# peterrum/dealii-multigrid

Hardware: AMD Instinct MI355X
Metric: DoF/s per V-cycle, 3D octant p=4 (higher is better)
Workload: dtype f64; 1 GPU; 3D octant (GeometryType quadrant) HMG-global p=4 FP64, NRefGlobal=8, SmootherDegree=3, coarse solver direct, f=1, zero Dirichlet (BASELINE.json configs[2]); n_dofs=137199985, n_cells=2127189, n_levels=9, parallelism=1 GPU, chebyshev_start_vector=deal.II's (i mod 11) - mean on the local numbering, fused_transfer_bricks=33509

## Files before the change

### dealii_multigrid_amd/__init__.py

```python
from __future__ import annotations

import ctypes as C
import os

import numpy as np

_LIB_PATH = os.environ.get("MGAMD_LIBRARY") or os.path.join(os.path.dirname(os.path.abspath(__file__)), "lib", "libmgamd.so")
F64, F32 = 8, 4
AMG_MIN_SHARDED_ROWS_DEFAULT = 20000
INVALID_DOF = 0xFFFFFFFF
ALL_DIRICHLET = 0x3F


class MgamdError(RuntimeError):
    pass


class NoDeviceError(MgamdError):
    pass


def _load():
    if not os.path.exists(_LIB_PATH):
        raise MgamdError(
# ... 354 lines not shown
    def rhs_constant(self):
        b = np.zeros(self.n_dofs)
        _chk(_lib.mgamd_dofs_rhs_constant(self._h, _ptr(b)))
        return b

    def groups(self):
        return [(self.info.group_B[g], self.info.group_slots[g]) for g in range(self.info.n_groups)]

    def matrix(self):
        nnz = C.c_uint64()
        _chk(_lib.mgamd_dofs_matrix(self._h, C.byref(nnz), None, None, None))
        ptr, col, val = np.zeros(self.n_dofs + 1, np.uint32), np.zeros(nnz.value, np.uint32), np.zeros(nnz.value)
        _chk(_lib.mgamd_dofs_matrix(self._h, C.byref(nnz), _ptr(ptr), _ptr(col), _ptr(val)))
        return ptr, col, val

    def amg_setup_info(self):
        n, rows, nnz = C.c_uint32(), (C.c_uint32 * 32)(), (C.c_uint64 * 32)()
        _chk(_lib.mgamd_dofs_amg_setup_info(self._h, C.byref(n), rows, nnz, 32))
        return [(rows[l], nnz[l]) for l in range(n.value)]

    def amg_hierarchy(self) -> "AmgHostHierarchy":
        return AmgHostHierarchy(self)

    def cell_slots(self):
        grp, slot = np.zeros(self.info.n_cells, np.uint8), np.zeros(self.info.n_cells, np.uint32)
        _chk(_lib.mgamd_dofs_get_cell_slots(self._h, _ptr(grp), _ptr(slot)))
        return grp, slot

    def halo_plan(self):
        sz = (C.c_uint32 * 4)()
        _chk(_lib.mgamd_dofs_halo_sizes(self._h, sz))
        npeer, nsend, nsh, nc = (int(v) for v in sz)
        plan = dict(peers=np.zeros(npeer, np.int32), peer_offset=np.zeros(npeer + 1, np.uint32), pack_idx=np.zeros(nsend, np.uint32),
                    sh_tail=np.zeros(nsh, np.uint32), sh_ptr=np.zeros(nsh + 1, np.uint32), sh_src=np.zeros(nc, np.int32),
                    sh_owner_src=np.zeros(nsh, np.int32))
        if npeer:
            _chk(_lib.mgamd_dofs_halo_get(self._h, _ptr(plan["peers"]), _ptr(plan["peer_offset"]), _ptr(plan["pack_idx"]), _ptr(plan["sh_tail"]),
                                          _ptr(plan["sh_ptr"]), _ptr(plan["sh_src"]), _ptr(plan["sh_owner_src"])))
        return plan

    def __del__(self):
        if getattr(self, "_h", None) and _lib is not None:
            _lib.mgamd_dofs_destroy(self._h)
            self._h = None


# ... 216 lines not shown
    def rhs_boundary_flux(self, b: Vector, q):
        q = _flux_array(q)
        _chk(_lib.mgamd_level_op_rhs_boundary_flux(self._h, _ptr(q), b._h))

    def distribute(self, x: Vector, kind: int = 0):
        _chk(_lib.mgamd_level_op_distribute(self._h, kind, x._h))

    def rhs_dirichlet(self, b: Vector, g: Vector, include_mass: bool = True):
        _chk(_lib.mgamd_level_op_rhs_dirichlet(self._h, g._h, 1 if include_mass else 0, b._h))

    def distribute_values(self, x: Vector, g: Vector):
        _chk(_lib.mgamd_level_op_distribute_values(self._h, x._h, g._h))

    def estimate_error(self, u: Vector, q=None):
        eta = np.zeros(self.dofs.info.n_cells, np.float64)
        qa = None if q is None else _flux_array(q)
        _chk(_lib.mgamd_level_op_estimate_error(self._h, u._h, None if qa is None else _ptr(qa), _ptr(eta)))
        return eta

    def _estimator_info(self):
        b, t0, t1 = C.c_uint64(), C.c_double(), C.c_double()
        _chk(_lib.mgamd_debug_level_op_estimator_info(self._h, C.byref(b), C.byref(t0), C.byref(t1)))
        return b.value, t0.value, t1.value

    def get_system_matrix(self) -> "SparseMatrix":
        if self.dofs.mass_coefficient() != self.mass_coefficient():
            raise MgamdError(f"get_system_matrix: the mass coefficient of the DoFs ({self.dofs.mass_coefficient()}) was changed after this "
                             f"operator was built with {self.mass_coefficient()}; the assembled matrix would be another operator's")
        return SparseMatrix(self.ctx, self.dofs)

    def __del__(self):
        if getattr(self, "_h", None) and _lib is not None:
            _lib.mgamd_level_op_destroy(self._h)
            self._h = None


class PreconditionChebyshev:
    def __init__(self, op: Operator, degree=3, smoothing_range=20.0, eig_cg_n_iterations=20):
        self.op = op
        self._h = C.c_void_p()
        _chk(_lib.mgamd_cheb_create(op._h, degree, C.c_double(smoothing_range), eig_cg_n_iterations, C.byref(self._h)))

    def vmult(self, dst: Vector, src: Vector):
        _chk(_lib.mgamd_cheb_vmult(self._h, dst._h, src._h))

    def step(self, dst: Vector, src: Vector):
# ... 519 lines not shown
```

### dealii_multigrid_amd/csrc/c_api_device.hip

```cpp
#include "runtime.hpp"
#include "kernels_amg.hpp"
#include <cstdio>

using namespace mgamd;

#define REQUIRE(cond)                                    \
  if (!(cond))                                           \
  throw std::invalid_argument("null or invalid argument: " #cond)

extern "C" {

int
mgamd_ctx_create(int device, mgamd_ctx **out)
{
  MGAMD_TRY
  REQUIRE(out);
  auto *c = new mgamd_ctx;
  try
    {
      c->ctx = std::make_unique<Ctx>(device);
    }
  catch (...)
    {
      delete c;
// ... 426 lines not shown
int
mgamd_level_op_estimate_error(mgamd_level_op *op, const mgamd_vec *u, const double q[6], double *eta)
{
  MGAMD_TRY
  REQUIRE(op && u);
  op->op->estimate_error(*u, q, eta);
  MGAMD_CATCH
}

int
mgamd_debug_level_op_estimator_info(const mgamd_level_op *op, uint64_t *bytes, double *build_ms, double *kernel_ms)
{
  MGAMD_TRY
  REQUIRE(op);
  uint64_t b  = 0;
  double   t0 = 0.0, t1 = 0.0;
  op->op->estimator_info(b, t0, t1);
  if (bytes)
    *bytes = b;
  if (build_ms)
    *build_ms = t0;
  if (kernel_ms)
    *kernel_ms = t1;
  MGAMD_CATCH
}

int
mgamd_level_op_debug_stamps(mgamd_level_op *op, unsigned long long *out, uint64_t max_count, uint64_t *count)
{
  MGAMD_TRY
  REQUIRE(op && out && count);
  *count = op->op->read_debug_stamps(out, max_count);
  MGAMD_CATCH
}

int
mgamd_cheb_create(mgamd_level_op *op, unsigned degree, double smoothing_range, unsigned eig_cg_n_iterations, mgamd_cheb **out)
{
  MGAMD_TRY
  REQUIRE(op && out);
  auto *h = new mgamd_cheb;
  try
    {
      h->c.reset(make_chebyshev(op->op.get(), degree, smoothing_range, eig_cg_n_iterations));
    }
  catch (...)
// ... 720 lines not shown
```

### dealii_multigrid_amd/csrc/c_api_host.cpp

```cpp
#include "api_common.hpp"

using namespace mgamd;

namespace mgamd
{
  thread_local std::string g_last_error;
}

struct mgamd_amg_host
{
  AmgHierarchyHost H;
};

struct mgamd_amg_shard
{
  AmgHierarchyHost          H;
  unsigned                  n_sharded = 0;
  std::vector<AmgShardPlan> plans;
};

extern "C" {

const char *
mgamd_last_error(void)
// ... 800 lines not shown
  std::vector<uint32_t> g, l;
  ls_copy_indices(*active_mesh_dofs->tables, *level_dofs->tables, (int)level, g, l);
  *count = g.size();
  if (global_idx)
    std::copy(g.begin(), g.end(), global_idx);
  if (level_idx)
    std::copy(l.begin(), l.end(), level_idx);
  MGAMD_CATCH
}

int
mgamd_dofs_get_cell_slots(const mgamd_dofs *d, uint8_t *group, uint32_t *slot)
{
  MGAMD_TRY
  if (!d || !group || !slot)
    throw std::invalid_argument("null argument");
  const LevelTables &L = *d->tables;
  std::copy(L.cell_group.begin(), L.cell_group.end(), group);
  std::copy(L.cell_slot.begin(), L.cell_slot.end(), slot);
  MGAMD_CATCH
}

int
mgamd_dofs_get_keys(const mgamd_dofs *d, int32_t *keys)
{
  MGAMD_TRY
  if (!d || !keys)
    throw std::invalid_argument("null argument");
  std::vector<DofKey> k;
  d->tables->export_dof_keys(k);
  static_assert(sizeof(DofKey) == 5 * sizeof(int32_t), "DofKey layout");
  std::memcpy(keys, k.data(), k.size() * sizeof(DofKey));
  MGAMD_CATCH
}

int
mgamd_dofs_get_cell_dofs(const mgamd_dofs *d, uint32_t *out)
{
  MGAMD_TRY
  if (!d || !out)
    throw std::invalid_argument("null argument");
  std::vector<uint32_t> v;
  d->tables->export_cell_dofs(v);
  std::memcpy(out, v.data(), v.size() * sizeof(uint32_t));
  MGAMD_CATCH
}
// ... 264 lines not shown
```

### dealii_multigrid_amd/csrc/kernels_apply.hpp

```cpp
#pragma once
#include "kernels_common.hpp"

namespace mgamd
{
#ifdef MGAMD_KERNEL_DEBUG
#define MGAMD_STAMP(k)                         \
  if (args.stamps && tid == 0)                 \
    args.stamps[(size_t)block * 8 + (k)] = wall_clock64();
#define MGAMD_ABLATED(bit) (args.ablate & (bit))
#define MGAMD_STAMP_OWNER(w)                   \
  if (args.stamps && tid == 0)                 \
    args.stamps[(size_t)block * 8 + 7] = (w) + 1;
#else
#define MGAMD_STAMP(k)
#define MGAMD_STAMP_OWNER(w)
#define MGAMD_ABLATED(bit) false
#endif

  template <typename T, int P>
  __device__ __forceinline__ void
  interior_diag_terms(const Mats<P, T> &mats, const int t, T &s_K, T &s_M)
  {
    const int tt[3] = {t % P, (t / P) % P, t / (P * P)};
    T         m[3], k[3];
// ... 337 lines not shown
        return (x % P) + P * ((y % P) + P * (z % P));
      }
      __device__ __forceinline__ void
      next()
      {
        constexpr int DZ = BLOCK / (NI * NI), DY = (BLOCK % (NI * NI)) / NI, DX = BLOCK % NI;
        x += DX;
        if (x > NI)
          {
            x -= NI;
            ++y;
          }
        y += DY;
        if (y > NI)
          {
            y -= NI;
            ++z;
          }
        z += DZ;
      }
    };
    const InteriorWalk walk0{tid % NI + 1, (tid / NI) % NI + 1, tid / (NI * NI) + 1};
    auto has_entry = [&](int it) -> bool { return (it + 1) * BLOCK <= G::N_INT || tid + it * BLOCK < G::N_INT; };
    int spos[ITERS];
#pragma unroll
    for (int it = 0; it < ITERS; ++it)
      {
        const int idx = tid + it * BLOCK;
        spos[it]      = idx < G::N_SHELL ? (int)args.g.shell_pos[idx] : -1;
      }
    if (sched.active && tid == 0)
      sched.publish(drawn, ticket_word);
    __syncthreads();

    constexpr bool x_from_b = MODE == MODE_CHEB_FIRST;
    auto load_tables = [&](uint32_t s, uint32_t &slot, uint32_t &base, uint32_t(&sg)[ITERS], double &h, uint32_t &fm, uint32_t &fl,
                           uint32_t(&cg)[ITC]) {
      slot = s;
      base = args.g.interior_base[slot];
      h    = args.g.h[slot];
      fm   = 0;
      fl   = 0;
      if constexpr (FUSE)
        {
          fl = args.fused.flags[(size_t)slot * BLOCK + tid];
          const uint32_t *__restrict__ c0 = args.fused.coarse_idx + (size_t)slot * NC3;
#pragma unroll
          for (int it = 0; it < ITC; ++it)
            cg[it] = NT_LOAD(c0 + min(tid + it * BLOCK, NC3 - 1));
        }
      if constexpr (brick_may_be_constrained(B, CONSTR))
        if (args.g.fmask != nullptr)
          fm = args.g.fmask[slot];
      const uint32_t *__restrict__ p0 = args.g.shell_idx + (size_t)slot * G::N_SHELL;
#pragma unroll
      for (int it = 0; it < ITERS; ++it)
        {
          if ((it + 1) * BLOCK <= G::N_SHELL)
            sg[it] = NT_LOAD(p0 + it * BLOCK + tid);
          else
            sg[it] = NT_LOAD(p0 + min(tid + it * BLOCK, G::N_SHELL - 1));
        }
    };
    auto load_values = [&](uint32_t base, const uint32_t(&sg)[ITERS], const uint32_t fl, const uint32_t(&cg)[ITC], T(&xv)[ITER], T(&sv)[ITERS],
                           T(&sbv)[ITERS], T(&cv)[ITC]) {
      const T *__restrict__ in = x_from_b ? args.epi.b : args.src;
#pragma unroll
      for (int it = 0; it < ITER; ++it)
        xv[it] = NT_LOAD(&in[base + (uint32_t)(has_entry(it) ? tid + it * BLOCK : 0)]);
#pragma unroll
      for (int it = 0; it < ITERS; ++it)
        {
          const uint32_t gi = sg[it] < args.gather_limit ? sg[it] : 0;
          sv[it]            = in[gi];
          if (x_from_b)
            sbv[it] = args.epi.dinv[gi];
          if (FUSE_R)
            sbv[it] = args.epi.b[((fl >> (2 * it)) & 1u) ? gi : 0];
        }
      if constexpr (FUSE_P)
        {
#pragma unroll
          for (int it = 0; it < ITC; ++it)
            cv[it] = args.fused.coarse[cg[it] != DEV_INVALID ? cg[it] : 0];
        }
    };

    uint32_t slot, base, sgi[ITERS], fmcur, flcur, cgi[ITC];
    double   hcur;
    T        xg[ITER], sval[ITERS], sb[ITERS], cval[ITC];
    load_tables(xcd_contiguous(w, n), slot, base, sgi, hcur, fmcur, flcur, cgi);
    load_values(base, sgi, flcur, cgi, xg, sval, sb, cval);

    for (;;)
      {
        const uint32_t block = slot;
        (void)block;
        uint32_t   vn       = slot;
        const bool has_next = sched.active && sched.take(ticket_word, vn);
        if (has_next && tid == 0)
          drawn = sched.draw();
        MGAMD_STAMP(0)
        MGAMD_STAMP_OWNER(w)
        const T rh = T(1) / T(hcur);
        if constexpr (MASS && is_cheb(MODE))
          {
            const T c = T(args.sigma) * T(args.g.q[slot]);
            for (int t = tid; t < P3; t += BLOCK)
              {
                T s_K, s_M;
                interior_diag_terms<T, P>(args.m, t, s_K, s_M);
                const T sv   = s_K + c * s_M;
                dtab[t]      = sv;
                dtab[P3 + t] = T(1) / sv;
              }
            if (x_from_b)
              __syncthreads();
          }
        auto interior_dinv = [&](int t) -> T {
          return fabs((double)dtab[t]) > 1.0e-10 * fabs((double)rh) ? rh * dtab[P3 + t] : T(1);
        };
        const bool fused_slot = FUSE && ((__builtin_amdgcn_readfirstlane((int)flcur) >> 15) & 1);
        T          bv[ITER], xo[ITER];
        uint32_t slotn = slot, basen = base, sgn[ITERS], fmn = fmcur, fln = flcur, cgn[ITC];
        double   hn = hcur;
        if (has_next)
          load_tables(vn, slotn, basen, sgn, hn, fmn, fln, cgn);
        {
#pragma unroll
          for (int it = 0; it < ITER; ++it)
            {
              const uint32_t g = base + (uint32_t)(has_entry(it) ? tid + it * BLOCK : 0);
              xo[it]           = T(0);
              bv[it]           = x_from_b ? xg[it] : T(0);
              if (MODE == MODE_CHEB && !FUSE_P && args.epi.xold)
                xo[it] = NT_LOAD(&args.epi.xold[g]);
              if ((MODE == MODE_RESIDUAL || is_cheb(MODE)) && !x_from_b)
                bv[it] = NT_LOAD(&args.epi.b[g]);
            }
        }
        if constexpr (FUSE_P)
          if (fused_slot)
            {
#pragma unroll
              for (int it = 0; it < ITC; ++it)
                if (tid + it * BLOCK < NC3)
                  bufA[tid + it * BLOCK] = ((flcur >> (16 + it)) & 1u) ? T(0) : cval[it];
              __syncthreads();
              T cin[NC], cout[G::N];
              for (int l = tid; l < NC * NC; l += BLOCK)
// ... 14 lines not shown
#pragma unroll
                  for (int i = 0; i < NC; ++i)
                    cin[i] = bufB[b0 + i * G::N];
                  line_embed_sym<T, P, BC>(args.fused.Eh, cin, cout);
#pragma unroll
                  for (int i = 0; i < G::N; ++i)
                    bufB[b0 + i * G::N] = cout[i];
                }
              __syncthreads();
              for (int l = tid; l < G::N * G::N; l += BLOCK)
                {
                  const int b0 = l * G::N;
#pragma unroll
                  for (int i = 0; i < NC; ++i)
                    cin[i] = bufB[b0 + i];
                  line_embed_sym<T, P, BC>(args.fused.Eh, cin, cout);
#pragma unroll
                  for (int i = 0; i < G::N; ++i)
                    bufB[b0 + i] = cout[i];
                }
              __syncthreads();
#pragma unroll
              for (int it = 0; it < ITERS; ++it)
                if (spos[it] >= 0 && sgi[it] < args.gather_limit)
                  {
                    const uint32_t f2 = (flcur >> (2 * it)) & 3u;
                    if (!(f2 & 2u))
                      sval[it] += bufB[spos[it]];
                    if (f2 & 1u)
                      args.fused.scratch[sgi[it]] = sval[it];
                  }
              InteriorWalk wk = walk0;
#pragma unroll
              for (int it = 0; it < ITER; ++it, wk.next())
                if (has_entry(it))
                  {
                    xg[it] += bufB[wk.pos()];
                    NT_STORE(xg[it], &args.fused.x_inout[base + (uint32_t)(tid + it * BLOCK)]);
                  }
            }
        if (x_from_b)
          {
#pragma unroll
            for (int it = 0; it < ITERS; ++it)
              sval[it] = args.epi.c0 * sb[it] * sval[it];
          }
#pragma unroll
        for (int it = 0; it < ITERS; ++it)
          if (spos[it] >= 0)
            bufA[spos[it]] = sgi[it] < args.gather_limit ? sval[it] : T(0);
        {
          InteriorWalk wk = walk0;
#pragma unroll
          for (int it = 0; it < ITER; ++it, wk.next())
            if (has_entry(it))
              bufA[wk.pos()] = x_from_b ? args.epi.c0 * interior_dinv(wk.type()) * bv[it] : xg[it];
        }
        __syncthreads();
        if (has_next && tid == 0)
          sched.publish(drawn, ticket_word);
        MGAMD_STAMP(1)

        bool any_hanging = false;
        if constexpr (brick_may_be_constrained(B, CONSTR))
          {
            any_hanging = fmcur != 0;
            if (any_hanging)
              brick_constraint_passes<T, P, B, BLOCK>(bufA, args.m, tid, 1, args.g.fmask + slot, false, &fmcur);
          }
        if constexpr (MODE == MODE_MASS)
          mass_sweeps<T, P, B, BLOCK, true, true, false>(bufA, args.m, tid, 1, &hcur, false);
        else
          lattice_sweeps<T, P, B, BLOCK, NoHook, true, (MODE != MODE_CHEB || sizeof(T) == 4), false, MASS>(
            bufA, bufB, args.m, tid, 1, &hcur, NoHook(), false, args.sigma, args.g.q + slot);
        if constexpr (brick_may_be_constrained(B, CONSTR))
          if (any_hanging)
            brick_constraint_passes<T, P, B, BLOCK>(bufA, args.m, tid, 1, args.g.fmask + slot, true, &fmcur);
        MGAMD_STAMP(2)

        T xgn[ITER], svaln[ITERS], sbn[ITERS], cvaln[ITC];
        if (has_next)
          load_values(basen, sgn, fln, cgn, xgn, svaln, sbn, cvaln);

        if (FUSE_R && fused_slot)
          {
            if constexpr (FUSE_R)
              {
                InteriorWalk wk = walk0;
#pragma unroll
                for (int it = 0; it < ITER; ++it, wk.next())
                  if (has_entry(it))
                    bufA[wk.pos()] = bv[it] - bufA[wk.pos()];
#pragma unroll
                for (int it = 0; it < ITERS; ++it)
                  if (spos[it] >= 0)
                    bufA[spos[it]] = sgi[it] < args.scatter_limit ? (((flcur >> (2 * it)) & 1u) ? sb[it] : T(0)) - bufA[spos[it]] : T(0);
                __syncthreads();
                T rin[G::N], rout[NC];
                for (int l = tid; l < G::N * G::N; l += BLOCK)
                  {
                    const int b0 = l * G::N;
#pragma unroll
                    for (int i = 0; i < G::N; ++i)
                      rin[i] = bufA[b0 + i];
                    line_embed_sym_T<T, P, BC>(args.fused.Eh, rin, rout);
#pragma unroll
                    for (int i = 0; i < NC; ++i)
                      bufA[b0 + i] = rout[i];
                  }
                __syncthreads();
                for (int l = tid; l < NC * G::N; l += BLOCK)
                  {
                    const int b0 = (l / NC) * G::N * G::N + l % NC;
#pragma unroll
                    for (int i = 0; i < G::N; ++i)
                      rin[i] = bufA[b0 + i * G::N];
                    line_embed_sym_T<T, P, BC>(args.fused.Eh, rin, rout);
#pragma unroll
                    for (int i = 0; i < NC; ++i)
// ... 30 lines not shown
                  T              r;
                  if (MODE == MODE_VMULT || MODE == MODE_MASS)
                    r = ax;
                  else if (MODE == MODE_RESIDUAL)
                    r = bv[it] - ax;
                  else
                    {
                      const T dv  = interior_dinv(wk.type());
                      const T xov = MODE == MODE_CHEB_SECOND ? args.epi.c0 * dv * bv[it] : xo[it];
                      const T xv  = x_from_b ? args.epi.c0 * dv * bv[it] : xg[it];
                      if (FUSE_P)
                        r = xv + args.epi.f2 * dv * (bv[it] - ax);
                      else
                        r = xv + args.epi.f1 * (xv - xov) + args.epi.f2 * dv * (bv[it] - ax);
                    }
                  if (MODE == MODE_CHEB && !FUSE_P)
                    store_result(args.epi, g, r);
                  else
                    NT_STORE(r, &args.epi.out[g]);
                }
            MGAMD_STAMP(3)
#pragma unroll
            for (int it = 0; it < ITERS; ++it)
              if (spos[it] >= 0 && sgi[it] < args.scatter_limit)
                atomic_add(&args.tail_acc[sgi[it] - args.n_interior], bufA[spos[it]]);
          }
        MGAMD_STAMP(4)
        if (!has_next)
          break;
        slot  = slotn;
        base  = basen;
        hcur  = hn;
        fmcur = fmn;
        flcur = fln;
#pragma unroll
        for (int it = 0; it < ITC; ++it)
          {
            cgi[it]  = cgn[it];
            cval[it] = cvaln[it];
          }
#pragma unroll
        for (int it = 0; it < ITERS; ++it)
          {
            sgi[it]  = sgn[it];
            sval[it] = svaln[it];
            sb[it]   = sbn[it];
          }
#pragma unroll
// ... 878 lines not shown
```

### dealii_multigrid_amd/csrc/kernels_common.hpp

```cpp
#pragma once
#include <hip/hip_runtime.h>
#include <stdint.h>

namespace mgamd
{
  constexpr uint32_t DEV_INVALID = 0xFFFFFFFFu;

  constexpr size_t KERNARG_LIMIT     = 4096;
  constexpr int    MAX_KERNEL_DEGREE = 7;

#ifndef MGAMD_NO_NT_STREAMS
#define NT_LOAD(p) __builtin_nontemporal_load(p)
#define NT_STORE(v, p) __builtin_nontemporal_store(v, p)
#else
#define NT_LOAD(p) (*(p))
#define NT_STORE(v, p) (*(p) = (v))
#endif

  __device__ __forceinline__ uint32_t
  xcd_contiguous(uint32_t b, uint32_t n)
  {
    const uint32_t k = b & 7u, q = n >> 3, r = n & 7u;
    return k * q + (k < r ? k : r) + (b >> 3);
  }
// ... 76 lines not shown
  persistent_brick(int p)
  {
    return 16 % p == 0 ? 16 / p : 0;
  }
  template <typename T, int P, int B>
  constexpr size_t
  apply_lds_bytes()
  {
    using G = Geo<P, B>;
    static_assert(persistent_lattice(G::N) == (G::SPW == 1 && G::N_INT > 0 && G::ROUNDS > 1), "persistent_lattice() and Geo disagree");
    return (2 * (size_t)G::SPW * G::N3 + 2 * P * P * P * (P == 1 ? G::SPW : 1) + G::SPW) * sizeof(T);
  }

  struct SlotGroupDev
  {
    const uint32_t *interior_base;
    const uint32_t *shell_idx;
    const uint16_t *mask;
    const double   *h;
    const uint16_t *shell_pos;
    uint32_t        n_slots;
    const uint32_t *fmask;
    const double   *q;
  };

  enum ApplyMode
  {
    MODE_VMULT    = 0,
    MODE_RESIDUAL = 1,
    MODE_CHEB     = 2,
    MODE_INVDIAG  = 3,
    MODE_CHEB_FIRST  = 4,
    MODE_CHEB_SECOND = 5,
    MODE_RESIDUAL_RESTRICT = 6,
    MODE_CHEB_PROLONGATE = 7,
    MODE_MASS = 8
  };
  constexpr int
  base_mode(int mode)
  {
    return mode == MODE_RESIDUAL_RESTRICT ? MODE_RESIDUAL : (mode == MODE_CHEB_PROLONGATE ? MODE_CHEB : mode);
  }

  template <typename T>
  struct Epilogue
  {
    T       *out;
// ... 1046 lines not shown
```

### dealii_multigrid_amd/csrc/level_operator.hpp

```cpp
#pragma once
#include "runtime.hpp"
#include "kernels.hpp"

#include <chrono>
#include <cmath>
#include <cstring>
#include <map>
#include <mutex>
#include <type_traits>
#include <unordered_map>

namespace mgamd
{
  inline int
  grid_for(size_t n)
  {
    size_t g = (n + 255) / 256;
    if (g > 2048)
      g = 2048;
    if (g < 1)
      g = 1;
    return (int)g;
  }

// ... 96 lines not shown
      }
    else if constexpr (persistent_lattice(G::N))
      {
        void (*kern)(ApplyArgs<T, P>) = lattice_apply_persistent_kernel<T, P, B, MODE, CONSTR, false>;
        if constexpr (MODE != MODE_MASS)
          if (a.sigma != 0.0)
            kern = lattice_apply_persistent_kernel<T, P, B, MODE, CONSTR, true>;
        launch_persistent(ctx, st, kern, grid, persistent_wgs_per_cu<T, P>(), G::ABLOCK, apply_lds_bytes<T, P, B>(), a, grid_cap);
      }
    else
      launch_lds(ctx, st, lattice_apply_kernel<T, P, B, MODE, CONSTR>, grid, G::ABLOCK, apply_lds_bytes<T, P, B>(), a);
    HIP_CHECK(hipGetLastError());
  }

  template <typename T>
  struct GroupDev
  {
    int            B = 1, N = 2;
    bool           constrained = false;
    size_t         n_halo      = 0;
    size_t         n_slots = 0;
    DBuf<uint32_t> interior_base, shell_idx;
    DBuf<uint16_t> mask, shell_pos;
    DBuf<double>   h, q, h_cell;
    DBuf<uint32_t> fmask;
    void
    upload_scales(const SlotGroup &g)
    {
      std::vector<double> ah(g.h.size()), ratio(g.h.size());
      bool                any = false;
      for (size_t s = 0; s < g.h.size(); ++s)
        {
          ah[s]    = g.a[s] * g.h[s];
          ratio[s] = g.h[s] * g.h[s] / g.a[s];
          any |= g.a[s] != 1.0;
        }
      h.upload(ah);
      q.upload(ratio);
      if (any)
        h_cell.upload(g.h);
    }
    const double *
    scale(bool mass_pass) const
    {
      return mass_pass && h_cell.p ? h_cell.p : h.p;
    }
    SlotGroupDev
    view(bool mass_pass) const
    {
      return SlotGroupDev{interior_base.p, shell_idx.p, mask.p, scale(mass_pass), shell_pos.p, (uint32_t)n_slots, fmask.p, q.p};
    }
    SlotGroupDev
    view(size_t begin, size_t end, bool mass_pass) const
    {
      const size_t n_shell = (size_t)N * N * N - (size_t)(N - 2) * (N - 2) * (N - 2);
      return SlotGroupDev{interior_base.p + begin, shell_idx.p + begin * n_shell, mask.p + begin, scale(mass_pass) + begin, shell_pos.p,
                          (uint32_t)(end - begin), fmask.p ? fmask.p + begin : nullptr, q.p + begin};
    }
    DBuf<uint32_t> uniq_ptr, uniq_idx;
    DBuf<uint16_t> loc;
    uint32_t       max_uniq = 0;
    bool
    has_clusters() const
    {
      return uniq_ptr.p != nullptr;
    }
    CellClusterDev
    cluster_view(bool mass_pass) const
    {
      return CellClusterDev{uniq_ptr.p, uniq_idx.p, loc.p, mask.p, scale(mass_pass), (uint32_t)n_slots, max_uniq, q.p};
    }
    size_t
    cluster_lds_bytes() const
    {
      return 2 * (size_t)std::max<uint32_t>(max_uniq, 1) * sizeof(T);
    }
    void
    build_clusters(const SlotGroup &g)
    {
      const size_t          ns = g.n_slots(), ncl = (ns + CLUSTER_CELLS - 1) / CLUSTER_CELLS;
// ... 161 lines not shown
          halo->sh_tail.upload(halo_plan->sh_tail);
          halo->sh_ptr.upload(halo_plan->sh_ptr);
          halo->sh_src.upload(halo_plan->sh_src);
          halo->sh_owner_src.upload(halo_plan->sh_owner_src);
          halo->send.alloc(std::max<size_t>(halo_plan->pack_idx.size(), 1));
          halo->recv.alloc(std::max<size_t>(halo_plan->pack_idx.size(), 1));
        }
      size_t best = 0;
      for (const SlotGroup &g : tables->groups)
        {
          auto d     = std::make_unique<GroupDev<T>>();
          d->B           = g.B;
          d->N           = g.N;
          d->constrained = g.constrained_group;
          d->n_halo      = g.n_halo_slots;
          d->n_slots = g.n_slots();
          if (d->n_slots)
            {
              d->interior_base.upload(g.interior_base);
              d->shell_idx.upload(g.shell_idx);
              d->mask.upload(g.mask);
              d->upload_scales(g);
              d->shell_pos.upload(g.shell_pos);
              if (std::any_of(g.fmask.begin(), g.fmask.end(), [](uint32_t m) { return m != 0; }))
                d->fmask.upload(g.fmask);
              if (p == 1 && g.B == 1 && !tables->ls_level)
                d->build_clusters(g);
            }
          const size_t work = d->n_slots * (size_t)g.N * g.N * g.N;
          if (work > best)
            {
              best       = work;
              dominant_B = g.B;
            }
          groups.push_back(std::move(d));
        }
      if (const char *e = getenv("MGAMD_ABLATE"))
        ablate = (uint32_t)atoi(e);
      if (const char *e = getenv("MGAMD_STAMP_B"))
        dominant_B = atoi(e);
      halo_overlap = getenv("MGAMD_NO_HALO_OVERLAP") == nullptr;
      if (const char *e = getenv("MGAMD_STAMPS"))
        {
          stamp_mode = atoi(e);
          size_t nwg = 0;
          for (auto &g : groups)
// ... 736 lines not shown
      float ms = 0.f;
      HIP_CHECK(hipEventElapsedTime(&ms, estimator->e0, estimator->e1));
      estimator->kernel_ms = ms;
    }
    void
    estimator_info(uint64_t &bytes, double &build_ms, double &kernel_ms) const override
    {
      bytes     = estimator ? estimator->bytes : 0;
      build_ms  = estimator ? estimator->build_ms : 0.0;
      kernel_ms = estimator ? estimator->kernel_ms : 0.0;
    }

    size_t
    read_debug_stamps(unsigned long long *out, size_t max_count) override
    {
      ctx->sync();
      const size_t n = std::min(max_count, stamps.n);
      if (n)
        HIP_CHECK(hipMemcpy(out, stamps.p, n * sizeof(unsigned long long), hipMemcpyDeviceToHost));
      return n;
    }

    void
    compute_inverse_diagonal(mgamd_vec &d) override
    {
      if (d.n != n_dofs())
        throw std::invalid_argument("compute_inverse_diagonal: vector size mismatch");
      Epilogue<T> e{d.as<T>(), nullptr, nullptr, nullptr, nullptr, T(0), T(0)};
      apply<MODE_VMULT>(nullptr, e, true);
    }
  };

}
```

### dealii_multigrid_amd/csrc/level_tables.hpp

```cpp
#pragma once
#include <algorithm>
#include <array>
#include <cmath>
#include <cstdlib>
#include <cstring>
#include "fe1d.hpp"
#include "octree.hpp"

#include <map>

namespace mgamd
{
  struct SharedInfo
  {
    uint64_t others  = 0;
    uint64_t regular = 0;
  };
  inline int
  shared_owner(const SharedInfo &si)
  {
    return __builtin_ctzll(si.regular);
  }
}

// ... 31 lines not shown
    s += M * N;
    if (y == N - 1)
      return s + (z - 1) * N + x;
    s += M * N;
    if (x == 0)
      return s + (z - 1) * M + (y - 1);
    s += M * M;
    return s + (z - 1) * M + (y - 1);
  }

  struct SlotGroup
  {
    int                   B = 1, N = 2, n_interior = 0, n_shell = 8;
    std::vector<uint32_t> interior_base;
    std::vector<uint32_t> shell_idx;
    std::vector<uint16_t> mask;
    std::vector<uint32_t> fmask;
    std::vector<double>   h;
    std::vector<double>   a;
    std::vector<uint32_t> first_cell;
    std::vector<uint16_t> shell_pos;
    uint32_t n_halo_slots = 0;
    bool constrained_group = false;
    size_t
    n_slots() const
    {
      return interior_base.size();
    }
  };

  struct DofKey
  {
    int32_t px, py, pz, dirmask, level;
  };

  inline uint64_t
  pack_key(uint32_t px, uint32_t py, uint32_t pz, int dm, int level)
  {
    return ((uint64_t)px << 43) | ((uint64_t)py << 25) | ((uint64_t)pz << 7) | ((uint64_t)dm << 4) | (uint64_t)(dm ? level : 0);
  }
  inline DofKey
  unpack_key(uint64_t k)
  {
    return DofKey{(int32_t)(k >> 43), (int32_t)((k >> 25) & 0x3ffff), (int32_t)((k >> 7) & 0x3ffff), (int32_t)((k >> 4) & 7),
                  (int32_t)(k & 15)};
  }

  inline void
  interpolate_hanging(const FE1D &fe, uint16_t mask, double *v, bool transpose)
  {
    if (!(mask >> MASK_FACE_SHIFT))
      return;
// ... 1281 lines not shown
                  perm.push_back((uint32_t)sl);
              auto permute = [&](auto &v, size_t width) {
                if (v.empty())
                  return;
                auto old = v;
                for (size_t n2 = 0; n2 < ns; ++n2)
                  std::copy(old.begin() + perm[n2] * width, old.begin() + (perm[n2] + 1) * width, v.begin() + n2 * width);
              };
              permute(g.interior_base, 1);
              permute(g.shell_idx, (size_t)g.n_shell);
              permute(g.mask, 1);
              permute(g.fmask, 1);
              permute(g.h, 1);
              permute(g.a, 1);
              permute(g.first_cell, 1);
              std::vector<uint32_t> new_of_old(ns);
              for (size_t n2 = 0; n2 < ns; ++n2)
                new_of_old[perm[n2]] = (uint32_t)n2;
              for (size_t ci = 0; ci < nc; ++ci)
                if (cell_group[ci] == gi)
                  cell_slot[ci] = new_of_old[cell_slot[ci]];
            }
        }
      build_robin_faces();
      build_dirichlet_cells();
    }

    void
    dirichlet_lift_add(const double *g, bool include_mass, double alpha, std::vector<double> &b) const
    {
      const int           n = p + 1, n3 = n * n * n;
      std::vector<double> xg(n3), lift(n3);
      for (size_t e = 0; e < dirichlet_cells.size(); ++e)
        {
          const uint32_t *idx = &dirichlet_cells.idx[e * n3];
          for (int t = 0; t < n3; ++t)
            xg[t] = is_dirichlet_index(idx[t]) ? g[idx[t]] : 0.0;
          const uint16_t mask = dirichlet_cells.mask[e];
          const double   ah = dirichlet_cells.scale[2 * e], h = dirichlet_cells.scale[2 * e + 1];
          interpolate_hanging(fe, mask, xg.data(), false);
          cell_stiffness_apply(ah, xg.data(), lift.data());
          if (include_mass && sigma != 0.0)
            cell_mass_add(h, sigma, xg.data(), lift.data());
          interpolate_hanging(fe, mask, lift.data(), true);
          for (int t = 0; t < n3; ++t)
            if (idx[t] < first_constrained())
// ... 82 lines not shown
```

### dealii_multigrid_amd/csrc/runtime.hpp

```cpp
#pragma once
#include "api_common.hpp"
#include "comm.hpp"

#include <hip/hip_runtime.h>

#include <functional>
#include <map>
#include <sstream>

namespace mgamd
{
#define HIP_CHECK(expr)                                                                                       \
  do                                                                                                          \
    {                                                                                                         \
      hipError_t e_ = (expr);                                                                                 \
      if (e_ != hipSuccess)                                                                                   \
        {                                                                                                     \
          std::ostringstream os_;                                                                             \
          os_ << "HIP error " << hipGetErrorString(e_) << " at " << __FILE__ << ":" << __LINE__ << ": " #expr; \
          throw std::runtime_error(os_.str());                                                                \
        }                                                                                                     \
    }                                                                                                         \
  while (0)

// ... 156 lines not shown
    }
    uint32_t
    n_dofs() const
    {
      return tables->n_dofs;
    }
    size_t
    n_dot() const
    {
      return comm ? (size_t)tables->n_interior + tables->n_tail_owned : (size_t)n_dofs();
    }
    virtual void
    vmult(mgamd_vec &dst, const mgamd_vec &src) = 0;
    virtual void
    vmult_mass(mgamd_vec &dst, const mgamd_vec &src) = 0;
    virtual void
    compute_inverse_diagonal(mgamd_vec &d) = 0;
    virtual void
    vmult_interface_up(mgamd_vec &dst, const mgamd_vec &src) = 0;
    virtual void
    vmult_interface_down(mgamd_vec &dst, const mgamd_vec &src) = 0;
    virtual size_t
    read_debug_stamps(unsigned long long *out, size_t max_count) = 0;
    void
    rhs(mgamd_vec &b, int kind = 0);
    void
    rhs_boundary_flux(mgamd_vec &b, const double q[6]);
    void
    distribute(mgamd_vec &x, int kind);
    virtual void
    rhs_dirichlet(mgamd_vec &rhs, const mgamd_vec &g, bool include_mass) = 0;
    virtual void
    distribute_values(mgamd_vec &x, const mgamd_vec &g) = 0;
    virtual void
    estimate_error(const mgamd_vec &u, const double *q, double *eta) = 0;
    virtual void
    estimator_info(uint64_t &bytes, double &build_ms, double &kernel_ms) const = 0;

  private:
    virtual void
    distribute_values_core(mgamd_vec &x, const mgamd_vec &g) = 0;
    void
    upload_load(mgamd_vec &b, const std::vector<double> &h);
  };

  struct ChebyshevBase
// ... 189 lines not shown
```

### include/mgamd_dev.h

```cpp
#ifndef MGAMD_DEV_H
#define MGAMD_DEV_H

#include "mgamd.h"

#ifdef __cplusplus
extern "C" {
#endif

int mgamd_level_op_debug_stamps(mgamd_level_op *op, unsigned long long *out, uint64_t max_count, uint64_t *count);

int mgamd_ctx_kernel_profile(mgamd_ctx *ctx, int enable);
int mgamd_ctx_kernel_profile_brick(mgamd_ctx *ctx, int brick_size);
int mgamd_ctx_kernel_profile_read(mgamd_ctx *ctx, double *total_ms, uint64_t *n_launches, double *algorithmic_bytes);
int mgamd_ctx_kernel_profile_bytes_moved(mgamd_ctx *ctx, double *bytes_moved);

int mgamd_debug_coarse_resolve(const char *name, uint64_t n_level0_dofs, int level0_sharded, int has_nested, int has_amg_global,
                               char used[32]);

typedef struct mgamd_amg_host mgamd_amg_host;
int mgamd_debug_amg_host_create(const mgamd_dofs *d, mgamd_amg_host **out);
int mgamd_debug_amg_host_destroy(mgamd_amg_host *h);
int mgamd_debug_amg_host_n_levels(const mgamd_amg_host *h, uint32_t *n_levels);
int mgamd_debug_amg_host_level_info(const mgamd_amg_host *h, uint32_t level, uint32_t *n_rows, uint64_t *nnz_A, uint32_t *n_cols_P,
                                    uint64_t *nnz_P, uint32_t *n_aggregates, double *lambda_max);
// ... 7 lines not shown
int mgamd_debug_amg_shard_match_rows(const mgamd_dofs *global, const mgamd_dofs *local, uint32_t *rows);
int mgamd_debug_amg_shard_n_levels(const mgamd_amg_shard *h, uint32_t *n_levels, uint32_t *n_sharded_levels);
int mgamd_debug_amg_shard_level_info(const mgamd_amg_shard *h, unsigned rank, uint32_t level, uint32_t info[12]);
int mgamd_debug_amg_shard_level_get(const mgamd_amg_shard *h, unsigned rank, uint32_t level, uint32_t *rows, uint32_t *ghost, int32_t *peers,
                                    uint32_t *peer_offset, uint32_t *send_count, uint32_t *recv_count, uint32_t *send_idx, uint32_t *A_ptr,
                                    uint32_t *A_col, double *A_val, uint32_t *P_ptr, uint32_t *P_col, double *P_val, uint32_t *R_ptr,
                                    uint32_t *R_col, double *R_val);

int mgamd_debug_csr_spmv(mgamd_ctx *ctx, int number_type, int mode, int lanes, uint32_t n_rows, uint32_t n_cols, const uint32_t *ptr,
                         const uint32_t *col, const double *val, const double *x, double *y, const double *b, const double *xold,
                         int xold_is_y, const double *dinv, double f1, double f2, int *lanes_used);

int mgamd_debug_csr_spmv_ex(mgamd_ctx *ctx, int number_type, int mode, int lanes, uint32_t n_rows, uint32_t n_cols, const uint32_t *ptr,
                            const uint32_t *col, const double *val, const double *x, double *y, const double *b, const double *xold,
                            int xold_is_y, const double *dinv, double f1, double f2, int max_blocks, int *lanes_used, int *blocks,
                            double *dot);
int mgamd_debug_csr_spmv_lanes_long(uint32_t n_rows, uint64_t nnz, int *lanes);
int mgamd_debug_matrix_time_spmv(mgamd_matrix *A, int mode, int lanes, unsigned reps, double *ms_per_launch);
int mgamd_debug_csr_row_pointers(uint32_t n_rows, const uint64_t *row_counts, uint32_t *ptr);

int mgamd_debug_tria_face_neighbours(const mgamd_tria *t, uint8_t *code, uint32_t *nbr);
int mgamd_debug_level_op_estimator_info(const mgamd_level_op *op, uint64_t *bytes, double *build_ms, double *kernel_ms);

#ifdef __cplusplus
}
#endif
#endif
```

Baseline: 15.26 billion DoF/s.

## Compress regular brick shell indices into per-entity run tables

For unconstrained bricks with N=17, a per-slot table of 26 entity base indices replaces the full per-DoF shell index list. Each lane reconstructs its global index through a ds_bpermute of the entity base plus a precomputed offset encoded in a per-position shell code. This cuts the index traffic that each brick reads from memory. In exchange it adds a lookahead on the scheduler ticket to learn whether the next slot is regular, some extra decode ALU work, and a fallback path for irregular slots.

```diff
diff --git a/dealii_multigrid_amd/__init__.py b/dealii_multigrid_amd/__init__.py
--- a/dealii_multigrid_amd/__init__.py
+++ b/dealii_multigrid_amd/__init__.py
@@ -400,6 +400,19 @@
     def amg_hierarchy(self) -> "AmgHostHierarchy":
         return AmgHostHierarchy(self)
 
+    def shell_runs(self, group: int):
+        ns, nr = C.c_uint32(), C.c_uint32()
+        _chk(_lib.mgamd_debug_dofs_shell_runs(self._h, group, C.byref(ns), C.byref(nr), None, None, None))
+        N = self.info.group_B[group] * self.degree + 1
+        n_shell = N ** 3 - (N - 2) ** 3 if N > 2 else N ** 3
+        idx = np.zeros((ns.value, n_shell), np.uint32)
+        if ns.value:
+            _chk(_lib.mgamd_debug_dofs_shell_runs(self._h, group, None, None, _ptr(idx), None, None))
+        code, runs = np.zeros(n_shell, np.uint32), np.zeros((ns.value, 32), np.uint32)
+        if _lib.mgamd_debug_dofs_shell_runs(self._h, group, None, None, None, _ptr(code), _ptr(runs)) != 0:
+            code = runs = None
+        return dict(n_slots=ns.value, n_regular=nr.value, shell_idx=idx, shell_code=code, shell_runs=runs)
+
     def cell_slots(self):
         grp, slot = np.zeros(self.info.n_cells, np.uint8), np.zeros(self.info.n_cells, np.uint32)
         _chk(_lib.mgamd_dofs_get_cell_slots(self._h, _ptr(grp), _ptr(slot)))
@@ -662,6 +675,9 @@
         b, t0, t1 = C.c_uint64(), C.c_double(), C.c_double()
         _chk(_lib.mgamd_debug_level_op_estimator_info(self._h, C.byref(b), C.byref(t0), C.byref(t1)))
         return b.value, t0.value, t1.value
+
+    def _set_shell_run(self, group: int, slot: int, word: int, value: int):
+        _chk(_lib.mgamd_debug_level_op_set_shell_run(self._h, group, slot, word, C.c_uint32(value)))
 
     def get_system_matrix(self) -> "SparseMatrix":
         if self.dofs.mass_coefficient() != self.mass_coefficient():
diff --git a/dealii_multigrid_amd/csrc/c_api_device.hip b/dealii_multigrid_amd/csrc/c_api_device.hip
--- a/dealii_multigrid_amd/csrc/c_api_device.hip
+++ b/dealii_multigrid_amd/csrc/c_api_device.hip
@@ -472,6 +472,15 @@
     *build_ms = t0;
   if (kernel_ms)
     *kernel_ms = t1;
+  MGAMD_CATCH
+}
+
+int
+mgamd_debug_level_op_set_shell_run(mgamd_level_op *op, unsigned group, uint32_t slot, unsigned word, uint32_t value)
+{
+  MGAMD_TRY
+  REQUIRE(op);
+  op->op->debug_set_shell_run(group, slot, word, value);
   MGAMD_CATCH
 }
 
diff --git a/dealii_multigrid_amd/csrc/c_api_host.cpp b/dealii_multigrid_amd/csrc/c_api_host.cpp
--- a/dealii_multigrid_amd/csrc/c_api_host.cpp
+++ b/dealii_multigrid_amd/csrc/c_api_host.cpp
@@ -846,6 +846,32 @@
 }
 
 int
+mgamd_debug_dofs_shell_runs(const mgamd_dofs *d, unsigned group, uint32_t *n_slots, uint32_t *n_regular, uint32_t *shell_idx, uint32_t *shell_code,
+                            uint32_t *shell_runs)
+{
+  MGAMD_TRY
+  if (!d)
+    throw std::invalid_argument("null argument");
+  const LevelTables &L = *d->tables;
+  if (group >= L.groups.size())
+    throw std::invalid_argument("shell_runs: no such slot group");
+  const SlotGroup &g = L.groups[group];
+  if (n_slots)
+    *n_slots = (uint32_t)g.n_slots();
+  if (n_regular)
+    *n_regular = (uint32_t)g.n_regular_slots();
+  if (shell_idx)
+    std::copy(g.shell_idx.begin(), g.shell_idx.end(), shell_idx);
+  if ((shell_code && g.shell_code.empty()) || (shell_runs && g.shell_runs.empty()))
+    throw std::invalid_argument("shell_runs: the group has no run tables (not a plain 17-point group)");
+  if (shell_code)
+    std::copy(g.shell_code.begin(), g.shell_code.end(), shell_code);
+  if (shell_runs)
+    std::copy(g.shell_runs.begin(), g.shell_runs.end(), shell_runs);
+  MGAMD_CATCH
+}
+
+int
 mgamd_dofs_get_keys(const mgamd_dofs *d, int32_t *keys)
 {
   MGAMD_TRY
diff --git a/dealii_multigrid_amd/csrc/kernels_apply.hpp b/dealii_multigrid_amd/csrc/kernels_apply.hpp
--- a/dealii_multigrid_amd/csrc/kernels_apply.hpp
+++ b/dealii_multigrid_amd/csrc/kernels_apply.hpp
@@ -383,20 +383,32 @@
     };
     const InteriorWalk walk0{tid % NI + 1, (tid / NI) % NI + 1, tid / (NI * NI) + 1};
     auto has_entry = [&](int it) -> bool { return (it + 1) * BLOCK <= G::N_INT || tid + it * BLOCK < G::N_INT; };
-    int spos[ITERS];
+    uint32_t scode[ITERS];
 #pragma unroll
     for (int it = 0; it < ITERS; ++it)
       {
         const int idx = tid + it * BLOCK;
-        spos[it]      = idx < G::N_SHELL ? (int)args.g.shell_pos[idx] : -1;
-      }
+        scode[it]     = idx < G::N_SHELL ? args.g.shell_code[idx] : 0x80000000u;
+      }
+    auto shell_word = [&](int it) -> uint32_t {
+      uint32_t v = scode[it];
+      asm volatile("" : "+v"(v));
+      return v;
+    };
+    auto has_shell = [&](int it) -> bool { return (it + 1) * BLOCK <= G::N_SHELL || (int)scode[it] >= 0; };
+    auto spos      = [&](int it) -> int { return (int)(shell_word(it) & 0xFFFFu); };
     if (sched.active && tid == 0)
       sched.publish(drawn, ticket_word);
     __syncthreads();
 
     constexpr bool x_from_b = MODE == MODE_CHEB_FIRST;
-    auto load_tables = [&](uint32_t s, uint32_t &slot, uint32_t &base, uint32_t(&sg)[ITERS], double &h, uint32_t &fm, uint32_t &fl,
-                           uint32_t(&cg)[ITC]) {
+    auto slot_regular = [&](const uint32_t s) -> bool {
+      using ConstWord = const uint32_t __attribute__((address_space(4)));
+      if (CONSTR || args.g.shell_runs == nullptr)
+        return false;
+      return *(ConstWord *)(uintptr_t)(args.g.shell_runs + (size_t)s * SHELL_RUN_STRIDE + SHELL_RUN_FLAG) == SHELL_RUN_REGULAR;
+    };
+    auto load_tables = [&](uint32_t s, uint32_t &slot, uint32_t &base, double &h, uint32_t &fm, uint32_t &fl, uint32_t(&cg)[ITC]) {
       slot = s;
       base = args.g.interior_base[slot];
       h    = args.g.h[slot];
@@ -404,15 +416,26 @@
       fl   = 0;
       if constexpr (FUSE)
         {
-          fl = args.fused.flags[(size_t)slot * BLOCK + tid];
+          int lane = tid;
+          asm volatile("" : "+v"(lane));
+          fl = args.fused.flags[(size_t)slot * BLOCK + lane];
           const uint32_t *__restrict__ c0 = args.fused.coarse_idx + (size_t)slot * NC3;
 #pragma unroll
           for (int it = 0; it < ITC; ++it)
-            cg[it] = NT_LOAD(c0 + min(tid + it * BLOCK, NC3 - 1));
+            cg[it] = NT_LOAD(c0 + min(lane + it * BLOCK, NC3 - 1));
         }
       if constexpr (brick_may_be_constrained(B, CONSTR))
         if (args.g.fmask != nullptr)
           fm = args.g.fmask[slot];
+    };
+    auto load_shell_tables = [&](const uint32_t slot, const bool regular, uint32_t(&sg)[ITERS]) {
+      if (regular)
+        {
+          uint32_t lane = (uint32_t)tid;
+          asm volatile("" : "+v"(lane));
+          sg[0] = args.g.shell_runs[(size_t)slot * SHELL_RUN_STRIDE + (lane & (SHELL_RUN_STRIDE - 1))];
+          return;
+        }
       const uint32_t *__restrict__ p0 = args.g.shell_idx + (size_t)slot * G::N_SHELL;
 #pragma unroll
       for (int it = 0; it < ITERS; ++it)
@@ -423,9 +446,20 @@
             sg[it] = NT_LOAD(p0 + min(tid + it * BLOCK, G::N_SHELL - 1));
         }
     };
-    auto load_values = [&](uint32_t base, const uint32_t(&sg)[ITERS], const uint32_t fl, const uint32_t(&cg)[ITC], T(&xv)[ITER], T(&sv)[ITERS],
-                           T(&sbv)[ITERS], T(&cv)[ITC]) {
+    auto load_values = [&](uint32_t base, uint32_t(&sg)[ITERS], const uint32_t fl, const uint32_t(&cg)[ITC], T(&xv)[ITER],
+                           T(&sv)[ITERS], T(&sbv)[ITERS], T(&cv)[ITC]) {
       const T *__restrict__ in = x_from_b ? args.epi.b : args.src;
+      if (!CONSTR && (uint32_t)__builtin_amdgcn_readlane((int)sg[0], SHELL_RUN_FLAG) == SHELL_RUN_REGULAR)
+        {
+          const int runs = (int)sg[0];
+#pragma unroll
+          for (int it = 0; it < ITERS; ++it)
+            {
+              const uint32_t c = shell_word(it);
+              const uint32_t b = (uint32_t)__builtin_amdgcn_ds_bpermute((int)((c >> 14) & 0x7Cu), runs);
+              sg[it]           = b != DEV_INVALID ? b + ((c >> 21) & 0xFFu) : DEV_INVALID;
+            }
+        }
 #pragma unroll
       for (int it = 0; it < ITER; ++it)
         xv[it] = NT_LOAD(&in[base + (uint32_t)(has_entry(it) ? tid + it * BLOCK : 0)]);
@@ -450,7 +484,14 @@
     uint32_t slot, base, sgi[ITERS], fmcur, flcur, cgi[ITC];
     double   hcur;
     T        xg[ITER], sval[ITERS], sb[ITERS], cval[ITC];
-    load_tables(xcd_contiguous(w, n), slot, base, sgi, hcur, fmcur, flcur, cgi);
+    load_tables(xcd_contiguous(w, n), slot, base, hcur, fmcur, flcur, cgi);
+    load_shell_tables(slot, slot_regular(slot), sgi);
+    bool reg_ahead = false;
+    {
+      uint32_t v = 0;
+      if (sched.active && sched.take(ticket_word, v))
+        reg_ahead = slot_regular(v);
+    }
     load_values(base, sgi, flcur, cgi, xg, sval, sb, cval);
 
     for (;;)
@@ -484,9 +525,12 @@
         const bool fused_slot = FUSE && ((__builtin_amdgcn_readfirstlane((int)flcur) >> 15) & 1);
         T          bv[ITER], xo[ITER];
         uint32_t slotn = slot, basen = base, sgn[ITERS], fmn = fmcur, fln = flcur, cgn[ITC];
-        double   hn = hcur;
+        double   hn   = hcur;
         if (has_next)
-          load_tables(vn, slotn, basen, sgn, hn, fmn, fln, cgn);
+          {
+            load_tables(vn, slotn, basen, hn, fmn, fln, cgn);
+            load_shell_tables(slotn, reg_ahead, sgn);
+          }
         {
 #pragma unroll
           for (int it = 0; it < ITER; ++it)
@@ -547,11 +591,11 @@
               __syncthreads();
 #pragma unroll
               for (int it = 0; it < ITERS; ++it)
-                if (spos[it] >= 0 && sgi[it] < args.gather_limit)
+                if (has_shell(it) && sgi[it] < args.gather_limit)
                   {
                     const uint32_t f2 = (flcur >> (2 * it)) & 3u;
                     if (!(f2 & 2u))
-                      sval[it] += bufB[spos[it]];
+                      sval[it] += bufB[spos(it)];
                     if (f2 & 1u)
                       args.fused.scratch[sgi[it]] = sval[it];
                   }
@@ -572,8 +616,8 @@
           }
 #pragma unroll
         for (int it = 0; it < ITERS; ++it)
-          if (spos[it] >= 0)
-            bufA[spos[it]] = sgi[it] < args.gather_limit ? sval[it] : T(0);
+          if (has_shell(it))
+            bufA[spos(it)] = sgi[it] < args.gather_limit ? sval[it] : T(0);
         {
           InteriorWalk wk = walk0;
 #pragma unroll
@@ -605,7 +649,11 @@
 
         T xgn[ITER], svaln[ITERS], sbn[ITERS], cvaln[ITC];
         if (has_next)
-          load_values(basen, sgn, fln, cgn, xgn, svaln, sbn, cvaln);
+          {
+            uint32_t v = 0;
+            reg_ahead  = sched.take(ticket_word, v) && slot_regular(v);
+            load_values(basen, sgn, fln, cgn, xgn, svaln, sbn, cvaln);
+          }
 
         if (FUSE_R && fused_slot)
           {
@@ -618,8 +666,11 @@
                     bufA[wk.pos()] = bv[it] - bufA[wk.pos()];
 #pragma unroll
                 for (int it = 0; it < ITERS; ++it)
-                  if (spos[it] >= 0)
-                    bufA[spos[it]] = sgi[it] < args.scatter_limit ? (((flcur >> (2 * it)) & 1u) ? sb[it] : T(0)) - bufA[spos[it]] : T(0);
+                  if (has_shell(it))
+                    {
+                      const int sp = spos(it);
+                      bufA[sp]     = sgi[it] < args.scatter_limit ? (((flcur >> (2 * it)) & 1u) ? sb[it] : T(0)) - bufA[sp] : T(0);
+                    }
                 __syncthreads();
                 T rin[G::N], rout[NC];
                 for (int l = tid; l < G::N * G::N; l += BLOCK)
@@ -696,8 +747,8 @@
             MGAMD_STAMP(3)
 #pragma unroll
             for (int it = 0; it < ITERS; ++it)
-              if (spos[it] >= 0 && sgi[it] < args.scatter_limit)
-                atomic_add(&args.tail_acc[sgi[it] - args.n_interior], bufA[spos[it]]);
+              if (has_shell(it) && sgi[it] < args.scatter_limit)
+                atomic_add(&args.tail_acc[sgi[it] - args.n_interior], bufA[spos(it)]);
           }
         MGAMD_STAMP(4)
         if (!has_next)
diff --git a/dealii_multigrid_amd/csrc/kernels_common.hpp b/dealii_multigrid_amd/csrc/kernels_common.hpp
--- a/dealii_multigrid_amd/csrc/kernels_common.hpp
+++ b/dealii_multigrid_amd/csrc/kernels_common.hpp
@@ -122,7 +122,11 @@
     uint32_t        n_slots;
     const uint32_t *fmask;
     const double   *q;
+    const uint32_t *shell_code = nullptr;
+    const uint32_t *shell_runs = nullptr;
   };
+  constexpr int      SHELL_RUN_STRIDE  = 32, SHELL_RUN_FLAG = 26;
+  constexpr uint32_t SHELL_RUN_REGULAR = 0xFFFFFFFEu;
 
   enum ApplyMode
   {
diff --git a/dealii_multigrid_amd/csrc/level_operator.hpp b/dealii_multigrid_amd/csrc/level_operator.hpp
--- a/dealii_multigrid_amd/csrc/level_operator.hpp
+++ b/dealii_multigrid_amd/csrc/level_operator.hpp
@@ -142,6 +142,10 @@
     size_t         n_slots = 0;
     DBuf<uint32_t> interior_base, shell_idx;
     DBuf<uint16_t> mask, shell_pos;
+    DBuf<uint32_t> shell_code, shell_runs;
+    static_assert(SHELL_RUN_STRIDE == SlotGroup::SHELL_RUN_STRIDE && SHELL_RUN_FLAG == SlotGroup::SHELL_RUN_FLAG &&
+                    SHELL_RUN_REGULAR == SlotGroup::SHELL_RUN_REGULAR,
+                  "kernel and host tables");
     DBuf<double>   h, q, h_cell;
     DBuf<uint32_t> fmask;
     void
@@ -168,14 +172,16 @@
     SlotGroupDev
     view(bool mass_pass) const
     {
-      return SlotGroupDev{interior_base.p, shell_idx.p, mask.p, scale(mass_pass), shell_pos.p, (uint32_t)n_slots, fmask.p, q.p};
+      return SlotGroupDev{interior_base.p, shell_idx.p, mask.p, scale(mass_pass), shell_pos.p, (uint32_t)n_slots, fmask.p, q.p,
+                          shell_code.p, shell_runs.p};
     }
     SlotGroupDev
     view(size_t begin, size_t end, bool mass_pass) const
     {
       const size_t n_shell = (size_t)N * N * N - (size_t)(N - 2) * (N - 2) * (N - 2);
       return SlotGroupDev{interior_base.p + begin, shell_idx.p + begin * n_shell, mask.p + begin, scale(mass_pass) + begin, shell_pos.p,
-                          (uint32_t)(end - begin), fmask.p ? fmask.p + begin : nullptr, q.p + begin};
+                          (uint32_t)(end - begin), fmask.p ? fmask.p + begin : nullptr, q.p + begin, shell_code.p,
+                          shell_runs.p ? shell_runs.p + begin * SHELL_RUN_STRIDE : nullptr};
     }
     DBuf<uint32_t> uniq_ptr, uniq_idx;
     DBuf<uint16_t> loc;
@@ -383,6 +389,10 @@
               d->mask.upload(g.mask);
               d->upload_scales(g);
               d->shell_pos.upload(g.shell_pos);
+              if (!g.shell_code.empty())
+                d->shell_code.upload(g.shell_code);
+              if (!g.shell_runs.empty())
+                d->shell_runs.upload(g.shell_runs);
               if (std::any_of(g.fmask.begin(), g.fmask.end(), [](uint32_t m) { return m != 0; }))
                 d->fmask.upload(g.fmask);
               if (p == 1 && g.B == 1 && !tables->ls_level)
@@ -1165,6 +1175,15 @@
     }
 
     void
+    debug_set_shell_run(unsigned group, uint32_t slot, unsigned word, uint32_t value) override
+    {
+      if (group >= groups.size() || !groups[group]->shell_runs.p || slot >= groups[group]->n_slots || word >= (unsigned)SHELL_RUN_STRIDE)
+        throw std::invalid_argument("debug_set_shell_run: no such word (group without run tables, slot or word out of range)");
+      ctx->sync();
+      HIP_CHECK(hipMemcpy(groups[group]->shell_runs.p + (size_t)slot * SHELL_RUN_STRIDE + word, &value, sizeof(value), hipMemcpyHostToDevice));
+    }
+
+    void
     compute_inverse_diagonal(mgamd_vec &d) override
     {
       if (d.n != n_dofs())
diff --git a/dealii_multigrid_amd/csrc/level_tables.hpp b/dealii_multigrid_amd/csrc/level_tables.hpp
--- a/dealii_multigrid_amd/csrc/level_tables.hpp
+++ b/dealii_multigrid_amd/csrc/level_tables.hpp
@@ -77,12 +77,89 @@
     std::vector<uint16_t> shell_pos;
     uint32_t n_halo_slots = 0;
     bool constrained_group = false;
+    static constexpr int      N_SHELL_ENTITIES = 26, SHELL_RUN_STRIDE = 32, SHELL_RUN_FLAG = 26;
+    static constexpr uint32_t SHELL_RUN_REGULAR = 0xFFFFFFFEu;
+    std::vector<uint32_t> shell_code, shell_runs;
     size_t
     n_slots() const
     {
       return interior_base.size();
     }
+    bool
+    slot_is_regular(size_t s) const
+    {
+      return !shell_runs.empty() && shell_runs[s * SHELL_RUN_STRIDE + SHELL_RUN_FLAG] == SHELL_RUN_REGULAR;
+    }
+    size_t
+    n_regular_slots() const
+    {
+      size_t n = 0;
+      for (size_t s = 0; s < n_slots(); ++s)
+        n += slot_is_regular(s);
+      return n;
+    }
   };
+
+  inline int
+  shell_entity_of(int N, int x, int y, int z)
+  {
+    auto      cls = [N](int v) { return v == 0 ? 0 : (v == N - 1 ? 2 : 1); };
+    const int e   = cls(x) + 3 * cls(y) + 9 * cls(z);
+    return e > 13 ? e - 1 : e;
+  }
+
+  inline int
+  shell_entity_stride(int N, bool along_x, bool along_y, bool along_z)
+  {
+    const int M = N - 2;
+    if (along_x + along_y + along_z == 2)
+      return along_x ? M + 1 : M;
+    return along_x ? 1 : M + 1;
+  }
+
+  inline void
+  build_shell_runs(SlotGroup &g)
+  {
+    g.shell_code.clear();
+    g.shell_runs.clear();
+    if (g.N != 17)
+      return;
+    constexpr int NE = SlotGroup::N_SHELL_ENTITIES, ST = SlotGroup::SHELL_RUN_STRIDE;
+    const int     M  = g.N - 2;
+    g.shell_code.resize(g.n_shell);
+    std::vector<int> ent(g.n_shell), off(g.n_shell), first(NE, -1), count(NE, 0);
+    for (int s = 0; s < g.n_shell; ++s)
+      {
+        const int  lin = g.shell_pos[s], x = lin % g.N, y = (lin / g.N) % g.N, z = lin / (g.N * g.N);
+        const bool ax = x > 0 && x < g.N - 1, ay = y > 0 && y < g.N - 1, az = z > 0 && z < g.N - 1;
+        ent[s]         = shell_entity_of(g.N, x, y, z);
+        const int rank = count[ent[s]]++;
+        const int st   = shell_entity_stride(g.N, ax, ay, az);
+        off[s]         = ax + ay + az == 2 ? (rank / M) * st + rank % M : rank * st;
+        if (first[ent[s]] < 0)
+          first[ent[s]] = s;
+        if (lin >= (1 << 16) || off[s] >= (1 << 8))
+          throw std::logic_error("shell_code: field overflow");
+        g.shell_code[s] = (uint32_t)lin | ((uint32_t)ent[s] << 16) | ((uint32_t)off[s] << 21);
+      }
+    if (g.constrained_group)
+      return;
+    g.shell_runs.assign(g.n_slots() * (size_t)ST, 0);
+    for (size_t sl = 0; sl < g.n_slots(); ++sl)
+      {
+        const uint32_t *idx  = &g.shell_idx[sl * (size_t)g.n_shell];
+        uint32_t       *runs = &g.shell_runs[sl * (size_t)ST];
+        for (int e = 0; e < NE; ++e)
+          runs[e] = idx[first[e]];
+        bool regular = true;
+        for (int s = 0; s < g.n_shell && regular; ++s)
+          {
+            const uint32_t b = runs[ent[s]];
+            regular          = idx[s] == (b == INVALID_DOF ? INVALID_DOF : b + (uint32_t)off[s]);
+          }
+        runs[SlotGroup::SHELL_RUN_FLAG] = regular ? SlotGroup::SHELL_RUN_REGULAR : 0u;
+      }
+  }
 
   struct DofKey
   {
@@ -1410,6 +1487,8 @@
                   cell_slot[ci] = new_of_old[cell_slot[ci]];
             }
         }
+      for (SlotGroup &g : groups)
+        build_shell_runs(g);
       build_robin_faces();
       build_dirichlet_cells();
     }
diff --git a/dealii_multigrid_amd/csrc/runtime.hpp b/dealii_multigrid_amd/csrc/runtime.hpp
--- a/dealii_multigrid_amd/csrc/runtime.hpp
+++ b/dealii_multigrid_amd/csrc/runtime.hpp
@@ -202,6 +202,8 @@
     vmult_interface_down(mgamd_vec &dst, const mgamd_vec &src) = 0;
     virtual size_t
     read_debug_stamps(unsigned long long *out, size_t max_count) = 0;
+    virtual void
+    debug_set_shell_run(unsigned group, uint32_t slot, unsigned word, uint32_t value) = 0;
     void
     rhs(mgamd_vec &b, int kind = 0);
     void
diff --git a/include/mgamd_dev.h b/include/mgamd_dev.h
--- a/include/mgamd_dev.h
+++ b/include/mgamd_dev.h
@@ -53,6 +53,10 @@
 int mgamd_debug_tria_face_neighbours(const mgamd_tria *t, uint8_t *code, uint32_t *nbr);
 int mgamd_debug_level_op_estimator_info(const mgamd_level_op *op, uint64_t *bytes, double *build_ms, double *kernel_ms);
 
+int mgamd_debug_dofs_shell_runs(const mgamd_dofs *d, unsigned group, uint32_t *n_slots, uint32_t *n_regular, uint32_t *shell_idx,
+                                uint32_t *shell_code, uint32_t *shell_runs);
+int mgamd_debug_level_op_set_shell_run(mgamd_level_op *op, unsigned group, uint32_t slot, unsigned word, uint32_t value);
+
 #ifdef __cplusplus
 }
 #endif
```

New measurement: 14.95 billion DoF/s. -2.0%, worse.
